# debbiemarkslab/BEAR

Measured on AMD Instinct MI355X. Metric: k-mer contexts/sec (DM-marginal+grad h), k=13, higher is better.
Workload: dtype f64

## Files before the change

### bear_amd/csrc/bear_count.hip

```cpp
#include <hip/hip_runtime.h>
#include <rocprim/device/device_radix_sort.hpp>
#include <rocprim/device/device_scan.hpp>
#include <stdint.h>

#include "../../include/bear_hip.h"
#include "bear_levels.h"

namespace {
thread_local int g_count_hip_error = 0;
#define CNT_TRY(expr)                    \
  do {                                   \
    hipError_t _e = (expr);              \
    if (_e != hipSuccess) {              \
      g_count_hip_error = (int)_e;       \
      st = BEAR_ERR_HIP;                 \
      goto done;                         \
    }                                    \
  } while (0)

template <int BITS, int W>
struct cnt_alphabet;
template <>
struct cnt_alphabet<3, 5> {
  static constexpr int MAX_LAG = 21;
// ... 288 lines not shown
  for (uint64_t i = (uint64_t)blockIdx.x * 256 + threadIdx.x; i < n; i += (uint64_t)gridDim.x * 256)
    flag[i] = (i == 0 || ((codes[i] ^ codes[i - 1]) & mask) != 0ull) ? 1u : 0u;
}
__global__ __launch_bounds__(256) void level_compact_kernel(const unsigned long long *__restrict__ codes, uint64_t n, unsigned long long mask,
                                                            unsigned long long fill, const uint32_t *__restrict__ flag,
                                                            uint32_t *__restrict__ scan_to_parent, unsigned long long *__restrict__ out_codes,
                                                            uint32_t *__restrict__ child_start, uint64_t n_runs) {
  for (uint64_t i = (uint64_t)blockIdx.x * 256 + threadIdx.x; i < n; i += (uint64_t)gridDim.x * 256) {
    const uint32_t run = scan_to_parent[i] - 1u;
    if (flag[i]) {
      out_codes[run] = (codes[i] & mask) | fill;
      child_start[run] = (uint32_t)i;
    }
    scan_to_parent[i] = run;
    if (i == 0) child_start[n_runs] = (uint32_t)n;
  }
}
}

namespace {
struct rec16 { unsigned long long a, b; };
struct rec16_less {
  __device__ __host__ bool operator()(const rec16 &x, const rec16 &y) const { return x.a < y.a || (x.a == y.a && x.b < y.b); }
};
template <typename T, typename Less>
int canonical_sort(T *d, uint64_t n, Less less, hipStream_t s) {
  int st = BEAR_OK;
  void *temp = nullptr;
  size_t tb = 0;
  T *out = nullptr;
  CNT_TRY(hipMalloc(&out, n * sizeof(T)));
  CNT_TRY(rocprim::merge_sort(nullptr, tb, d, out, n, less, s));
  CNT_TRY(hipMalloc(&temp, tb ? tb : 8));
  CNT_TRY(rocprim::merge_sort(temp, tb, d, out, n, less, s));
  CNT_TRY(hipMemcpyAsync(d, out, n * sizeof(T), hipMemcpyDeviceToDevice, s));
  CNT_TRY(hipStreamSynchronize(s));
done:
  if (temp) (void)hipFree(temp);
  if (out) (void)hipFree(out);
  return st;
}
}

int bear_canonical_order(void *records, uint64_t n, int width, hipStream_t s) {
  if (n < 2) return BEAR_OK;
  if (!records) return BEAR_ERR_INVALID_ARG;
  if (width == 16) return canonical_sort(static_cast<rec16 *>(records), n, rec16_less(), s);
  if (width == 8) return canonical_sort(static_cast<unsigned long long *>(records), n, rocprim::less<unsigned long long>(), s);
  if (width == 4) return canonical_sort(static_cast<uint32_t *>(records), n, rocprim::less<uint32_t>(), s);
  return BEAR_ERR_INVALID_ARG;
}

namespace {
__global__ __launch_bounds__(256) void window_keys_kernel(const unsigned long long *__restrict__ codes, uint64_t n, int shift, unsigned long long mask,
                                                          unsigned long long *__restrict__ keys, uint32_t *__restrict__ vals) {
  for (uint64_t i = (uint64_t)blockIdx.x * 256 + threadIdx.x; i < n; i += (uint64_t)gridDim.x * 256) {
    keys[i] = (codes[i] >> shift) & mask;
    vals[i] = (uint32_t)i;
  }
}
__global__ __launch_bounds__(256) void window_compact_kernel(const unsigned long long *__restrict__ keys, const uint32_t *__restrict__ perm, uint64_t n,
                                                             int shift, unsigned long long fill, const uint32_t *__restrict__ flag,
                                                             const uint32_t *__restrict__ scan, unsigned long long *__restrict__ out_codes,
                                                             uint32_t *__restrict__ child_start, uint32_t *__restrict__ row_of_context,
                                                             uint64_t n_runs) {
  for (uint64_t j = (uint64_t)blockIdx.x * 256 + threadIdx.x; j < n; j += (uint64_t)gridDim.x * 256) {
    const uint32_t run = scan[j] - 1u;
    if (flag[j]) {
      out_codes[run] = (keys[j] << shift) | fill;
      child_start[run] = (uint32_t)j;
    }
    row_of_context[perm[j]] = run;
    if (j == 0) child_start[n_runs] = (uint32_t)n;
  }
}
}

void bear_window_free(bear_window_dev *wt) {
  if (!wt) return;
  (void)hipFree(wt->codes);
  (void)hipFree(wt->row_of_context);
  (void)hipFree(wt->perm);
  (void)hipFree(wt->child_start);
  (void)hipFree(wt->rows);
  wt->codes = nullptr;
  wt->row_of_context = wt->perm = wt->child_start = nullptr;
  wt->rows = nullptr;
  wt->n = 0;
  wt->bytes = 0;
}

int bear_window_build(const unsigned long long *codes, uint64_t n_rows, int pos, int fw, bear_window_dev *out, hipStream_t s) {
  if (!codes || !out || n_rows == 0 || n_rows > 0xfffffffeull || pos < 0 || fw < 1 || pos + fw > 21) return BEAR_ERR_INVALID_ARG;
  int st = BEAR_OK;
  const int shift = 3 * pos;
  const unsigned long long mask = (1ull << (3 * fw)) - 1ull;
  unsigned long long fill = 0ull;
  for (int l = 0; l < 21; ++l)
    if (l < pos || l >= pos + fw) fill |= 5ull << (3 * l);
  unsigned long long *keys_in = nullptr, *keys = nullptr;
  uint32_t *vals_in = nullptr, *flag = nullptr, *scan = nullptr, n_runs = 0;
  void *temp = nullptr;
  size_t tb = 0, tb2 = 0;
  out->pos = pos;
  out->n = 0;
  out->codes = nullptr;
// ... 105 lines not shown
```

### bear_amd/csrc/bear_hip.hip

```cpp
#include "bear_host.h"
#include "kernels_finalize.h"
#include "kernels_rows.h"
#include "kernels_sorted.h"
#include "kernels_plan.h"
#include "kernels_synth.h"
#include "kernels_refmix.h"
#include "kernels_mixplan.h"
#include "kernels_sample.h"
#include "kernels_shuffle.h"
#include "kernels_refplan.h"

#ifdef PLN_STAMPS
#define PLN_DBG_ARG , ws->dbg
#else
#define PLN_DBG_ARG
#endif

thread_local int g_last_hip_error = 0;

extern "C" {

int bear_abi_version(void) { return BEAR_ABI_VERSION; }

const char *bear_strerror(int status) {
// ... 147 lines not shown
#define PRIOR_LAUNCH(AR, GRAD)                                                                                                          \
  hipLaunchKernelGGL((dm_prior_kernel<AR, GRAD>), dim3(grid), dim3(BEAR_THREADS), 0, s, counts, prior, n_rows, prm, grad_prior, \
                     reinterpret_cast<const double2 *>(ws->logtab), ws->partials)
    BEAR_DISPATCH_2(train_ar, grad_prior, PRIOR_LAUNCH);
#undef PRIOR_LAUNCH
  }
  HIP_TRY(hipGetLastError());
  hipLaunchKernelGGL(finalize_kernel, dim3(1), dim3(256), 0, s, ws->partials, grid, 2, out);
  HIP_TRY(hipGetLastError());
  return BEAR_OK;
}

int bear_dm_ref_f64(bear_ws *ws, const uint32_t *train, const uint32_t *ref, uint64_t n_rows,
                    double h_signed, double tau_signed, double nu_signed, double eps, int train_ar,
                    double *out, void *stream) {
  int st = check_ws(ws);
  if (st != BEAR_OK) return st;
  if (!out || (n_rows && (!train || !ref))) return BEAR_ERR_INVALID_ARG;
  if (misaligned(train) || misaligned(ref) || misaligned8(out)) return BEAR_ERR_INVALID_ARG;
  hipStream_t s = static_cast<hipStream_t>(stream);
  const bear_params prm = params_ref(h_signed, tau_signed, nu_signed, eps);
  const double2 *lt = reinterpret_cast<const double2 *>(ws->logtab);
  int grid = grid_rows(ws, n_rows);
  if (train_ar || getenv("BEAR_ROWS_KERNEL")) {
#define REF_LAUNCH(AR) hipLaunchKernelGGL((dm_ref_kernel<AR>), dim3(grid), dim3(BEAR_THREADS), 0, s, train, ref, n_rows, prm, lt, ws->partials)
    BEAR_DISPATCH_1(train_ar, REF_LAUNCH);
#undef REF_LAUNCH
  } else {
    grid = grid_sorted(ws, n_rows);
    hipLaunchKernelGGL(dm_ref_sorted_kernel, dim3(grid), dim3(SRT_THREADS), sizeof(srt_lds_r), s, train, ref, n_rows, prm, lt, ws->partials);
  }
  HIP_TRY(hipGetLastError());
  hipLaunchKernelGGL(finalize_kernel, dim3(1), dim3(256), 0, s, ws->partials, grid, 4, out);
  HIP_TRY(hipGetLastError());
  return BEAR_OK;
}

static void plan_free(bear_plan *p) {
  if (!p) return;
  (void)hipFree(p->tiles);
  (void)hipFree(p->stream);
  (void)hipFree(p->heavy_col);
  (void)hipFree(p->heavy_row);
  (void)hipFree(p->heavy_stop);
  (void)hipFree(p->hist);
  (void)hipFree(p->live);
  for (int k = 0; k < p->n_cnn_levels; ++k) bear_level_free(&p->cnn_levels[k]);
  for (int k = 0; k <= CNN_MAX_LAG; ++k)
    for (int q = 0; q < p->n_cnn_win[k]; ++q) bear_window_free(&p->cnn_win[k][q]);
  (void)hipFree(p->live2);
  (void)hipFree(p->tiles_p);
  (void)hipFree(p->tiles_u);
  (void)hipFree(p->ref_items);
  (void)hipFree(p->hist0_base);
  (void)hipFree(p->heavy0);
  (void)hipFree(p->sum0);
  delete p;
}

int bear_plan_create(bear_ws *ws, const uint32_t *counts, uint64_t n_rows, int ncol, bear_plan **out) {
  if (!out) return BEAR_ERR_INVALID_ARG;
  *out = nullptr;
  int st = check_ws(ws);
  if (st != BEAR_OK) return st;
  if ((ncol != 4 && ncol != 5) || (n_rows && !counts) || misaligned(counts)) return BEAR_ERR_INVALID_ARG;
  bear_plan *p = new (std::nothrow) bear_plan();
  if (!p) return BEAR_ERR_NOMEM;
  memset(p, 0, sizeof(*p));
  p->device = ws->device;
  p->ncol = ncol;
  p->n_rows = n_rows;
  p->counts = counts;
  hipError_t e = hipMalloc(&p->hist, sizeof(unsigned long long) * (2 * SRT_NKEY + PLN_NBIG + 1));
  if (e == hipSuccess) e = hipMemset(p->hist, 0, sizeof(unsigned long long) * (2 * SRT_NKEY + PLN_NBIG + 1));
  if (e != hipSuccess) {
    g_last_hip_error = (int)e;
    plan_free(p);
    return BEAR_ERR_HIP;
  }
  if (n_rows == 0) {
    *out = p;
    return BEAR_OK;
  }
  const uint64_t n_quads = (n_rows + PLN_QUAD - 1) / PLN_QUAD;
  uint8_t *d_quad = nullptr, *h_quad = nullptr;
  unsigned long long *d_cnt = nullptr;
  std::vector<pln_tile> tiles;
  e = hipMalloc(&d_quad, 3 * n_quads);
  if (e == hipSuccess) e = hipMalloc(&d_cnt, sizeof(unsigned long long) * 9);
  if (e == hipSuccess) e = hipMemset(d_cnt, 0, sizeof(unsigned long long) * 9);
  if (e == hipSuccess) {
    const int grid = grid_capped((n_quads + 255) / 256, (uint64_t)ws->num_cu * 8);
    hipLaunchKernelGGL(plan_scan_kernel, dim3(grid), dim3(256), 0, 0, counts, n_rows, ncol, d_quad, d_cnt, p->hist);
    e = hipGetLastError();
  }
  unsigned long long h_cnt[3] = {0, 0, 0}, h_total[3] = {0, 0, 0};
  if (e == hipSuccess) e = hipMemcpy(h_cnt, d_cnt, sizeof(h_cnt), hipMemcpyDeviceToHost);
  if (e == hipSuccess) e = hipMemcpy(h_total, d_cnt + 6, sizeof(h_total), hipMemcpyDeviceToHost);
  for (int k = 0; k < 3; ++k) p->count_total[k] = p->count_bound[k] = (double)h_total[k];
  uint64_t off16 = 0, n_tiles = 0;
  const char *cut_env = getenv("BEAR_PLAN_CUT");
  const bool host_cut = cut_env && cut_env[0] == 'h';
  if (e == hipSuccess && host_cut) {
    h_quad = (uint8_t *)malloc(3 * n_quads);
    if (!h_quad) e = hipErrorOutOfMemory;
    if (e == hipSuccess) e = hipMemcpy(h_quad, d_quad, 3 * n_quads, hipMemcpyDeviceToHost);
  }
  if (e == hipSuccess && host_cut) {
    uint64_t q = 0;
// ... 183 lines not shown

uint64_t bear_plan_tile_count(const bear_plan *plan) { return plan ? plan->n_tiles : 0; }

int bear_plan_tile_info(const bear_plan *plan, uint64_t first, uint64_t count, uint64_t *row0, uint32_t *rows, uint32_t *items,
                        uint64_t *stream_offset) {
  if (!plan || first + count > plan->n_tiles || (count && (!row0 || !rows || !items || !stream_offset))) return BEAR_ERR_INVALID_ARG;
  if (!count) return BEAR_OK;
  std::vector<pln_tile> h(count);
  int prev = 0;
  (void)hipGetDevice(&prev);
  (void)hipSetDevice(plan->device);
  const hipError_t e = hipMemcpy(h.data(), plan->tiles + first, sizeof(pln_tile) * count, hipMemcpyDeviceToHost);
  (void)hipSetDevice(prev);
  if (e != hipSuccess) {
    g_last_hip_error = (int)e;
    return BEAR_ERR_HIP;
  }
  for (uint64_t k = 0; k < count; ++k) {
    row0[k] = h[k].row0;
    rows[k] = h[k].rows_items >> 16;
    items[k] = h[k].rows_items & 0xffffu;
    stream_offset[k] = (uint64_t)h[k].off16 * 16;
  }
  return BEAR_OK;
}

int bear_plan_create_ref(bear_ws *ws, const uint32_t *train, const uint32_t *ref, uint64_t n_rows, bear_plan **out) {
  if (!out) return BEAR_ERR_INVALID_ARG;
  *out = nullptr;
  if ((n_rows && !ref) || misaligned(ref)) return BEAR_ERR_INVALID_ARG;
  bear_plan *p = nullptr;
  int st = bear_plan_create(ws, train, n_rows, 4, &p);
  if (st != BEAR_OK) return st;
  p->ref = ref;
  if (p->count_total[1] > 0.0 && (double)p->n_heavy[0] * 2.0 > p->count_total[1]) {
    (void)hipFree(p->tiles);
    (void)hipFree(p->stream);
    (void)hipFree(p->heavy_col);
    (void)hipFree(p->heavy_row);
    (void)hipFree(p->heavy_stop);
    p->tiles = nullptr;
    p->stream = nullptr;
    p->heavy_col = nullptr;
    p->heavy_row = nullptr;
    p->heavy_stop = nullptr;
    p->n_tiles = 0;
    p->n_heavy[0] = p->n_heavy[1] = p->n_heavy[2] = 0;
    p->rows_ref = 1;
    p->bytes = sizeof(unsigned long long) * (2 * SRT_NKEY + PLN_NBIG + 1);
    *out = p;
    return BEAR_OK;
  }
  unsigned long long *d_meta = nullptr;
  hipError_t e = hipMalloc(&d_meta, sizeof(unsigned long long) * 72);
  if (e == hipSuccess) e = hipMemset(d_meta, 0, sizeof(unsigned long long) * 72);
  if (e == hipSuccess) e = hipMalloc(&p->sum0, sizeof(double));
  if (e == hipSuccess) e = hipMemset(p->sum0, 0, sizeof(double));
  p->hist0_base = d_meta;
  unsigned long long h_meta[72];
  memset(h_meta, 0, sizeof(h_meta));
  const int grid = grid_capped((n_rows + 1023) / 1024, (uint64_t)ws->num_cu * 8);
  if (e == hipSuccess && n_rows) {
    hipLaunchKernelGGL(rpl_build_kernel, dim3(grid), dim3(256), 0, 0, train, ref, n_rows, 0, d_meta, d_meta + 32, d_meta + 64, p->sum0,
                       static_cast<rpl_item *>(nullptr), static_cast<uint32_t *>(nullptr));
    e = hipGetLastError();
    if (e == hipSuccess) e = hipMemcpy(h_meta, d_meta, sizeof(h_meta), hipMemcpyDeviceToHost);
  }
  if (e == hipSuccess) {
    unsigned long long run = 0, cur[RPL_NKEY];
    for (int k = 0; k < RPL_NKEY; ++k) {
      cur[k] = run;
      run += h_meta[k];
    }
    p->n_ref_items = run;
    p->n_heavy0 = h_meta[64];
    if (run) e = hipMalloc(&p->ref_items, sizeof(rpl_item) * run);
    if (e == hipSuccess && p->n_heavy0) e = hipMalloc(&p->heavy0, sizeof(uint32_t) * p->n_heavy0);
    if (e == hipSuccess) e = hipMemcpy(d_meta, cur, sizeof(cur), hipMemcpyHostToDevice);
    if (e == hipSuccess) e = hipMemset(d_meta + 64, 0, sizeof(unsigned long long));
    if (e == hipSuccess && n_rows && (run || p->n_heavy0)) {
      hipLaunchKernelGGL(rpl_build_kernel, dim3(grid), dim3(256), 0, 0, train, ref, n_rows, 1, d_meta, d_meta + 32, d_meta + 64, p->sum0,
                         p->ref_items, p->heavy0);
      e = hipGetLastError();
    }
    if (e == hipSuccess) e = hipDeviceSynchronize();
#ifdef BEAR_DET_BUILD
    for (int k = 0; k < RPL_NKEY && e == hipSuccess; ++k)
      if (bear_canonical_order(p->ref_items + cur[k], h_meta[k], 16, 0) != BEAR_OK) e = hipErrorUnknown;
    if (e == hipSuccess && bear_canonical_order(p->heavy0, p->n_heavy0, 4, 0) != BEAR_OK) e = hipErrorUnknown;
#endif
  }
  if (e != hipSuccess) {
    g_last_hip_error = (int)e;
    plan_free(p);
    return e == hipErrorOutOfMemory ? BEAR_ERR_NOMEM : BEAR_ERR_HIP;
  }
  p->hist0 = d_meta + 32;
  p->bytes += sizeof(rpl_item) * p->n_ref_items + sizeof(uint32_t) * p->n_heavy0 + sizeof(unsigned long long) * 72;
  *out = p;
  return BEAR_OK;
}

static int launch_prior_plan(bear_ws *ws, const bear_plan *plan, const double *prior, uint64_t n_rows, const bear_params &prm,
                             const double *theta, int train_ar, int prior_normalized, double *out, hipStream_t s) {
  const int grid = grid_plan(ws, plan->n_tiles);
  const double2 *lt = reinterpret_cast<const double2 *>(ws->logtab);
  const bear_step_io io = ws_io(ws, theta, BEAR_THETA_NET, out);
  if (train_ar)
    hipLaunchKernelGGL((dm_prior_plan_kernel<true, true>), dim3(grid), dim3(PLN_THREADS), sizeof(pln_lds_n), s, prior, n_rows, prm,
                       plan_view(plan), lt, ws->partials, io PLN_DBG_ARG);
  else if (prior_normalized)
    hipLaunchKernelGGL((dm_prior_plan_kernel<true, false>), dim3(grid), dim3(PLN_THREADS), sizeof(pln_lds_n), s, prior, n_rows, prm,
                       plan_view(plan), lt, ws->partials, io PLN_DBG_ARG);
  else
    hipLaunchKernelGGL((dm_prior_plan_kernel<false, false>), dim3(grid), dim3(PLN_THREADS), sizeof(pln_lds_n), s, prior, n_rows, prm,
                       plan_view(plan), lt, ws->partials, io PLN_DBG_ARG);
  HIP_TRY(hipGetLastError());
  return BEAR_OK;
}

int bear_dm_prior_plan_f64(bear_ws *ws, const bear_plan *plan, const uint32_t *counts, const double *prior,
                           uint64_t n_rows, double h_signed, double eps, int train_ar, int prior_normalized,
                           double *out, void *stream) {
  int st = check_ws(ws);
  if (st != BEAR_OK) return st;
  if (!plan || !out || (n_rows && (!counts || !prior))) return BEAR_ERR_INVALID_ARG;
  if (check_plan_step(ws, plan, counts, n_rows, 5, true) != BEAR_OK || misaligned(prior) || misaligned8(out)) return BEAR_ERR_INVALID_ARG;
  const bear_params prm = params_net(h_signed, eps);
  if (plan_is_rows(plan)) return launch_prior_rows(ws, plan, prior, prm, nullptr, train_ar, out, nullptr, static_cast<hipStream_t>(stream));
  return launch_prior_plan(ws, plan, prior, n_rows, prm, nullptr, train_ar, prior_normalized, out, static_cast<hipStream_t>(stream));
}

int launch_prior_plan_grad(bear_ws *ws, const bear_plan *plan, const double *prior, const bear_params &prm,
                                  const double *theta, int train_ar, int prior_normalized, double *out, double *grad_prior,
                                  hipStream_t s) {
  const int grid = grid_plan(ws, plan->n_tiles);
  const double2 *lt = reinterpret_cast<const double2 *>(ws->logtab);
  const pln_view pv = plan_view(plan);
  const bear_step_io io = ws_io(ws, theta, BEAR_THETA_NET, out);
  if (train_ar)
    hipLaunchKernelGGL((dm_prior_plan_grad_kernel<true, true>), dim3(grid), dim3(PLN_THREADS), sizeof(pln_lds_g), s, prior, prm, pv, lt,
                       grad_prior, ws->partials, io);
  else if (prior_normalized)
    hipLaunchKernelGGL(dm_prior_plan_grad_inplace_kernel, dim3(grid), dim3(PLN_THREADS), sizeof(pln_lds_gi), s, prior, prm, pv, lt,
                       grad_prior, ws->partials, io);
  else
    hipLaunchKernelGGL((dm_prior_plan_grad_kernel<false, false>), dim3(grid), dim3(PLN_THREADS), sizeof(pln_lds_g), s, prior, prm, pv, lt,
                       grad_prior, ws->partials, io);
  HIP_TRY(hipGetLastError());
  auto fixup_grid = [&](uint64_t nh) { return grid_capped((nh + 255) / 256, (uint64_t)ws->num_cu * 8); };
#define FIXUP(NORM, AR, ROWS, N) \
// ... 44 lines not shown
int bear_dm_refmix_plan_grad_f64(bear_ws *ws, const bear_plan *plan, const uint32_t *counts, const double *net_rows,
                                 const double *ref_rows, uint64_t n_rows, const double *h_signed_dev, const double *tau_signed_dev,
                                 const double *net_weight_signed_dev, double eps, int train_ar, double *out, double *grad_net_rows,
                                 void *stream) {
  int st = check_ws(ws);
  if (st != BEAR_OK) return st;
  if (!plan || !out || !h_signed_dev || !tau_signed_dev || !net_weight_signed_dev) return BEAR_ERR_INVALID_ARG;
  if (n_rows && (!counts || !net_rows || !ref_rows || !grad_net_rows)) return BEAR_ERR_INVALID_ARG;
  if (check_plan_step(ws, plan, counts, n_rows, 5) != BEAR_OK) return BEAR_ERR_INVALID_ARG;
  if (misaligned(net_rows) || misaligned(ref_rows) || misaligned(grad_net_rows) || misaligned8(out) || misaligned8(h_signed_dev) ||
      misaligned8(tau_signed_dev) || misaligned8(net_weight_signed_dev) || !(eps >= 0.0))
    return BEAR_ERR_INVALID_ARG;
  hipStream_t s = static_cast<hipStream_t>(stream);
  const int grid = grid_plan(ws, plan->n_tiles);
  const double2 *lt = reinterpret_cast<const double2 *>(ws->logtab);
  const pln_view pv = plan_view(plan);
  const bear_step_io io = ws_io(ws, nullptr, BEAR_THETA_REF, out);
#define MIX_LAUNCH(AR)                                                                                                            \
  hipLaunchKernelGGL(dm_refmix_plan_grad_kernel<AR>, dim3(grid), dim3(PLN_THREADS), sizeof(pln_lds_g), s, net_rows, ref_rows, \
                     h_signed_dev, tau_signed_dev, net_weight_signed_dev, eps, pv, lt, grad_net_rows, ws->partials, io)
  BEAR_DISPATCH_1(train_ar, MIX_LAUNCH);
#undef MIX_LAUNCH
  HIP_TRY(hipGetLastError());
  if (pv.n_heavy_col + pv.n_heavy_row) {
    const uint64_t nh = pv.n_heavy_col + pv.n_heavy_row;
    const int g2 = grid_capped((nh + 255) / 256, (uint64_t)ws->num_cu * 4);
#define MIX_FIXUP(AR)                                                                                                      \
  hipLaunchKernelGGL(dm_refmix_fixup_kernel<AR>, dim3(g2), dim3(256), 0, s, net_rows, ref_rows, h_signed_dev, tau_signed_dev, \
                     net_weight_signed_dev, eps, pv, lt, grad_net_rows)
    BEAR_DISPATCH_1(train_ar, MIX_FIXUP);
#undef MIX_FIXUP
    HIP_TRY(hipGetLastError());
  }
  return BEAR_OK;
}


static int launch_ref_plan(bear_ws *ws, const bear_plan *plan, const uint32_t *ref, uint64_t n_rows, const bear_params &prm,
                           const double *theta, int train_ar, double *out, hipStream_t s, const bear_apply_io &apply = NO_APPLY) {
  const double2 *lt = reinterpret_cast<const double2 *>(ws->logtab);
  const bear_step_io io = ws_io(ws, theta, BEAR_THETA_REF, out);
  int grid;
  if (plan->rows_ref) {
    if (plan->ref != ref) return BEAR_ERR_INVALID_ARG;
    grid = grid_dense(ws, n_rows);
#define REF_ROWS(AR) \
  hipLaunchKernelGGL(dm_ref_rows_kernel<AR>, dim3(grid), dim3(BEAR_THREADS), 0, s, plan->counts, ref, n_rows, prm, lt, ws->partials, io, apply)
    BEAR_DISPATCH_1(train_ar, REF_ROWS);
#undef REF_ROWS
  } else if (plan->ref) {
    if (plan->ref != ref) return BEAR_ERR_INVALID_ARG;
    rpl_view rv;
    rv.items = plan->ref_items;
    rv.n_items = plan->n_ref_items;
    rv.hist0 = plan->hist0;
    rv.heavy0 = plan->heavy0;
    rv.n_heavy0 = plan->n_heavy0;
    rv.sum0 = plan->sum0;
    const uint64_t units = (plan->n_ref_items + 63) / 64, want = (units + 3) / 4 + 2, cap = (uint64_t)ws->num_cu * (units > 131072 ? 6 : 4);
    grid = grid_capped(want, cap);
#define REF_ITEMS(AR) \
  hipLaunchKernelGGL(dm_ref_items_kernel<AR>, dim3(grid), dim3(256), 0, s, prm, rv, plan_view(plan), lt, ws->partials, io, apply)
    BEAR_DISPATCH_1(train_ar, REF_ITEMS);
#undef REF_ITEMS
  } else {
    grid = grid_plan(ws, plan->n_tiles);
#define REF_PLAN(AR)                                                                                                                     \
  hipLaunchKernelGGL(dm_ref_plan_kernel<AR>, dim3(grid), dim3(PLN_THREADS), sizeof(pln_lds_r), s, ref, n_rows, prm, plan_view(plan), lt, \
                     ws->partials, io, apply)
    BEAR_DISPATCH_1(train_ar, REF_PLAN);
#undef REF_PLAN
  }
  HIP_TRY(hipGetLastError());
  return BEAR_OK;
}

int bear_dm_ref_plan_f64(bear_ws *ws, const bear_plan *plan, const uint32_t *train, const uint32_t *ref,
                         uint64_t n_rows, double h_signed, double tau_signed, double nu_signed, double eps,
                         int train_ar, double *out, void *stream) {
  int st = check_ws(ws);
  if (st != BEAR_OK) return st;
  if (!plan || !out || (n_rows && (!train || !ref))) return BEAR_ERR_INVALID_ARG;
  if (check_plan_step(ws, plan, train, n_rows, 4) != BEAR_OK || misaligned(ref) || misaligned8(out)) return BEAR_ERR_INVALID_ARG;
  return launch_ref_plan(ws, plan, ref, n_rows, params_ref(h_signed, tau_signed, nu_signed, eps), nullptr, train_ar, out,
                         static_cast<hipStream_t>(stream));
}

static int ref_reduce(bear_ws *ws, const bear_plan *plan, const uint32_t *train, const uint32_t *ref, uint64_t n_rows, const double *theta,
                      double eps, int train_ar, double *packed, hipStream_t s, const bear_apply_io &apply) {
  int st = check_ws(ws);
  if (st != BEAR_OK) return st;
  if (!plan || !packed || !theta || !n_rows || !train || !ref) return BEAR_ERR_INVALID_ARG;
  if (check_plan_step(ws, plan, train, n_rows, 4) != BEAR_OK || misaligned(ref) || misaligned8(packed)) return BEAR_ERR_INVALID_ARG;
  return launch_ref_plan(ws, plan, ref, n_rows, params_eps(eps), theta, train_ar, packed, s, apply);
}

int bear_ref_train_reduce_f64(bear_ws *ws, const bear_plan *plan, const uint32_t *train, const uint32_t *ref, uint64_t n_rows,
                              const double *theta, double eps, int train_ar, double *packed, void *stream) {
  return ref_reduce(ws, plan, train, ref, n_rows, theta, eps, train_ar, packed, static_cast<hipStream_t>(stream), NO_APPLY);
}

int bear_ref_train_step_f64(bear_ws *ws, const bear_plan *plan, const uint32_t *train, const uint32_t *ref, uint64_t n_rows,
                            double *theta, double *adam_m, double *adam_v, double *adam_t, double eps, int train_ar,
                            double learning_rate, double scale, double *out, double *loss_buf, uint64_t loss_cap, void *stream) {
  if (!adam_m || !adam_v || !adam_t) return BEAR_ERR_INVALID_ARG;
  hipStream_t s = static_cast<hipStream_t>(stream);
  if (two_launch_step()) {
    int st = ref_reduce(ws, plan, train, ref, n_rows, theta, eps, train_ar, out, s, NO_APPLY);
    if (st != BEAR_OK) return st;
    return launch_train_apply(theta, 3, out, adam_m, adam_v, adam_t, learning_rate, scale, train_ar, loss_buf, loss_cap, s);
  }
  return ref_reduce(ws, plan, train, ref, n_rows, theta, eps, train_ar, out, s,
// ... 207 lines not shown
```

### bear_amd/csrc/bear_host.h

```cpp
#pragma once
#include <hip/hip_runtime.h>
#include <math.h>
#include <stdint.h>
#include <stdlib.h>
#include <string.h>

#include <initializer_list>
#include <new>
#include <vector>

#include "bear_common.h"
#include "bear_levels.h"
#include "plan_common.h"

#define BEAR_INTERNAL __attribute__((visibility("hidden")))

static inline int check_ws(const bear_ws *ws) {
  if (!ws) return BEAR_ERR_INVALID_ARG;
  int dev = -1;
  if (hipGetDevice(&dev) != hipSuccess) return BEAR_ERR_NO_DEVICE;
  if (dev != ws->device) return BEAR_ERR_WRONG_DEVICE;
  return BEAR_OK;
}

// ... 88 lines not shown
                                       double scale, int train_ar, double *loss_buf, uint64_t loss_cap) {
  bear_apply_io A;
  A.theta = theta;
  A.m = adam_m;
  A.v = adam_v;
  A.t_state = adam_t;
  A.loss_buf = loss_buf;
  A.loss_cap = (unsigned long long)loss_cap;
  A.lr = learning_rate;
  A.scale = scale;
  A.n_theta = n_theta;
  A.train_ar = train_ar;
  return A;
}

static inline bool two_launch_step() {
  const char *e = getenv("BEAR_AMD_TWO_LAUNCH_STEP");
  return e && e[0] && e[0] != '0';
}

struct rpl_item;
struct bear_plan {
  int device;
  int ncol;
  uint64_t n_rows;
  const uint32_t *counts;
  pln_tile *tiles;
  unsigned char *stream;
  pln_heavy_col *heavy_col;
  pln_heavy_row *heavy_row;
  uint64_t *heavy_stop;
  unsigned long long *hist;
  uint16_t *live;
  uint64_t n_tiles;
  uint64_t n_heavy[3];
  int rows_ref;
  uint64_t n_live_rows;
  double count_total[3];
  double count_bound[3];
  uint64_t bytes;
  bear_level_dev cnn_levels[CNN_MAX_LAG];
  int n_cnn_levels, cnn_lag, cnn_fw;
  bear_window_dev cnn_win[CNN_MAX_LAG + 1][CNN_MAX_WIN];
  int n_cnn_win[CNN_MAX_LAG + 1];
  int n_cnn_windows;
  const uint64_t *cnn_codes;
  uint16_t *live2;
  pln_tile *tiles_p, *tiles_u;
  uint64_t n_tiles_p, n_tiles_u;
  const uint64_t *pair_codes;
  int pair_lag;
  const uint32_t *ref;
  rpl_item *ref_items;
  uint64_t n_ref_items, n_heavy0;
  unsigned long long *hist0;
  unsigned long long *hist0_base;
  uint32_t *heavy0;
  double *sum0;
};

static inline pln_view plan_view(const bear_plan *p) {
  pln_view v;
  v.tiles = p->tiles;
  v.stream = p->stream;
  v.heavy_col = p->heavy_col;
  v.heavy_row = p->heavy_row;
  v.heavy_stop = p->heavy_stop;
  v.hist = p->hist;
  v.hist_big = p->hist + 2 * SRT_NKEY;
  v.big_in_hist = 1;
  v.live = p->live;
  v.live2 = p->live2;
  v.subset = 0;
  v.n_tiles = p->n_tiles;
  v.n_heavy_col = p->n_heavy[0];
  v.n_heavy_row = p->n_heavy[1];
  v.n_heavy_stop = p->n_heavy[2];
  return v;
}

#define PLAN_ROWS 15
static inline bool plan_is_rows(const bear_plan *p) { return p->ncol == PLAN_ROWS; }
static inline int check_plan_step(const bear_ws *ws, const bear_plan *plan, const uint32_t *counts, uint64_t n_rows, int ncol,
                                  bool or_rows = false) {
  if (plan->ncol != ncol && !(or_rows && plan_is_rows(plan))) return BEAR_ERR_INVALID_ARG;
  if (plan->counts != counts || plan->n_rows != n_rows || plan->device != ws->device) return BEAR_ERR_INVALID_ARG;
  return BEAR_OK;
}

BEAR_INTERNAL int linear_ws_setup(bear_ws *ws);
BEAR_INTERNAL int cnn_ws_setup(bear_ws *ws);
BEAR_INTERNAL int eval_ws_setup(bear_ws *ws);

extern "C" {
BEAR_INTERNAL int launch_prior_plan_grad(bear_ws *ws, const bear_plan *plan, const double *prior, const bear_params &prm,
                                         const double *theta, int train_ar, int prior_normalized, double *out, double *grad_prior,
                                         hipStream_t s);
BEAR_INTERNAL int launch_train_apply(double *theta, int n_theta, const double *packed, double *adam_m, double *adam_v, double *adam_t,
                                     double learning_rate, double scale, int train_ar, double *loss_buf, uint64_t loss_cap, hipStream_t s);
}
```

### bear_amd/csrc/bear_levels.h

```cpp
#pragma once
#include <hip/hip_runtime.h>
#include <stdint.h>

#define CNN_MAX_LAG 21
#define CNN_MAX_WIN 6

struct bear_level_dev {
  uint64_t n;
  int letters;
  unsigned long long *codes;
  uint32_t *parent_of_below;
  uint32_t *child_start;
  double *rows;
  uint64_t bytes;
};

struct bear_window_dev {
  int pos;
  uint64_t n;
  unsigned long long *codes;
  uint32_t *row_of_context;
  uint32_t *perm;
  uint32_t *child_start;
  double *rows;
  uint64_t bytes;
};
int bear_window_build(const unsigned long long *codes, uint64_t n_rows, int pos, int fw, bear_window_dev *out, hipStream_t stream);
void bear_window_free(bear_window_dev *wt);

int bear_level_build(const unsigned long long *codes_below, uint64_t n_below, int letters, bear_level_dev *out, hipStream_t stream);
void bear_level_free(bear_level_dev *lv);

int bear_canonical_order(void *records, uint64_t n, int width, hipStream_t stream);
```

### bear_amd/csrc/kernels_refplan.h

```cpp
#pragma once
#include "kernels_plan.h"

#define RPL_NKEY 32
#define RPL_HEAVY_KEY 24

struct rpl_item {
  uint32_t c, rb;
  double R;
};
static_assert(sizeof(rpl_item) == 16, "one 16-byte lane load per record");

struct rpl_view {
  const rpl_item *items;
  uint64_t n_items;
  const unsigned long long *hist0;
  const uint32_t *heavy0;
  uint64_t n_heavy0;
  const double *sum0;
};

__global__ __launch_bounds__(256) void rpl_build_kernel(const uint32_t *__restrict__ train, const uint32_t *__restrict__ ref, uint64_t n_rows,
                                                        int fill, unsigned long long *__restrict__ bucket,
                                                        unsigned long long *__restrict__ hist0, unsigned long long *__restrict__ n_heavy0,
                                                        double *__restrict__ sum0, rpl_item *__restrict__ items,
                                                        uint32_t *__restrict__ heavy0) {
  constexpr int RPT = 4;
  __shared__ uint32_t s_bucket[RPL_NKEY], s_hist0[RPL_NKEY];
  __shared__ unsigned long long s_at[RPL_NKEY];
  __shared__ double s_sum;
  const uint32_t tid = threadIdx.x;
  const uint64_t per_block = (n_rows + gridDim.x - 1) / gridDim.x;
  const uint64_t r_begin = (uint64_t)blockIdx.x * per_block, r_end = r_begin + per_block < n_rows ? r_begin + per_block : n_rows;
  for (uint64_t base = r_begin; base < r_end; base += 256u * RPT) {
    if (tid < RPL_NKEY) s_bucket[tid] = s_hist0[tid] = 0u;
    if (tid == 0) s_sum = 0.0;
    __syncthreads();
    uint32_t c[RPT][4], rb[RPT][4], rank[RPT][4];
    double R[RPT];
    double my_sum = 0.0;
#pragma unroll
    for (int k = 0; k < RPT; ++k) {
      const uint64_t row = base + tid + 256u * k;
      R[k] = -1.0;
#pragma unroll
      for (int b = 0; b < 4; ++b) c[k][b] = rb[k][b] = rank[k][b] = 0u;
      if (row < r_end) {
        uint64_t rs = 0;
#pragma unroll
        for (int b = 0; b < 4; ++b) {
          c[k][b] = train[row * 5 + b];
          rb[k][b] = ref[row * 5 + b];
          rs += rb[k][b];
        }
        R[k] = (double)rs;
#pragma unroll
        for (int b = 0; b < 4; ++b) {
          if (c[k][b] == 0u) continue;
          if (rs == 0) {
            my_sum += (double)c[k][b];
            if (c[k][b] <= SRT_CL) {
              if (!fill) atomicAdd(&s_hist0[c[k][b] - 1], 1u);
            } else if (fill) {
              heavy0[atomicAdd(n_heavy0, 1ull)] = c[k][b];
            } else {
              atomicAdd(n_heavy0, 1ull);
            }
          } else {
            const uint32_t key = (c[k][b] > SRT_CL ? SRT_CL + 1u : c[k][b]) - 1u;
            rank[k][b] = atomicAdd(&s_bucket[key], 1u);
          }
        }
      }
    }
    if (!fill && my_sum != 0.0) atomicAdd(&s_sum, my_sum);
    __syncthreads();
    if (tid < RPL_NKEY && !fill) {
      if (s_bucket[tid]) atomicAdd(&bucket[tid], (unsigned long long)s_bucket[tid]);
      if (s_hist0[tid]) atomicAdd(&hist0[tid], (unsigned long long)s_hist0[tid]);
    }
    if (!fill && tid == 0 && s_sum != 0.0) atomicAdd(sum0, s_sum);
    if (fill) {
      if (tid < RPL_NKEY) s_at[tid] = s_bucket[tid] ? atomicAdd(&bucket[tid], (unsigned long long)s_bucket[tid]) : 0ull;
      __syncthreads();
#pragma unroll
      for (int k = 0; k < RPT; ++k) {
        if (!(R[k] > 0.0)) continue;
#pragma unroll
        for (int b = 0; b < 4; ++b) {
          if (c[k][b] == 0u) continue;
          const uint32_t key = (c[k][b] > SRT_CL ? SRT_CL + 1u : c[k][b]) - 1u;
          rpl_item it;
          it.c = c[k][b];
          it.rb = rb[k][b];
          it.R = R[k];
          items[s_at[key] + rank[k][b]] = it;
        }
      }
    }
    __syncthreads();
  }
}

template <bool AR>
__global__ __launch_bounds__(256) void dm_ref_items_kernel(bear_params prm_arg, rpl_view rv, pln_view pv, const double2 *__restrict__ logtab_g,
                                                           double *__restrict__ partials, const bear_step_io io, const bear_apply_io apply) {
  __shared__ double2 s_log[BEAR_LOGTAB_N];
  const bear_params prm = bear_params_of(prm_arg, io);
  const uint32_t tid = threadIdx.x, lane = tid & 63u;
  const double u = prm.inv_h, eps = prm.eps;
  const double A = u + 5.0 * eps;
  const double x4 = prm.nw * prm.V * u + eps;
  const double VU = prm.V * u;
  const double tau = prm.tau;
  const double w2c = tau * (eps + 0.25 * VU);
  const double nwV = prm.nw * prm.V;
  double acc[4] = {0.0, 0.0, 0.0, 0.0};
  if (tid < BEAR_LOGTAB_N) s_log[tid] = logtab_g[tid];
  __syncthreads();
  auto alpha_from = [&](double rb, double R) {
    const double dev = __builtin_fma(rb + eps, bear_rcp(R), -0.25);
    return __builtin_fma(__builtin_fma(prm.E, dev, 0.25), VU, eps);
  };
  auto accumulate = [&](double x, double m, const bear_dp &o) {
    const double w1 = eps - x, P = m * o.P;
    acc[0] = __builtin_fma(m, o.D, acc[0]);
    acc[1] = __builtin_fma(w1, P, acc[1]);
    acc[2] = __builtin_fma(__builtin_fma(-tau, x, w2c), P, acc[2]);
    acc[3] = __builtin_fma(nwV * w1, P, acc[3]);
  };
  auto accumulate_ar = [&](double rb, double R, double c) {
    const double dev = __builtin_fma(rb + eps, bear_rcp(R), -0.25);
    const double f = __builtin_fma(prm.E, dev, 0.25) * prm.V;
    const double p = f + eps;
    const double dLdf = c * bear_rcp(p);
    acc[0] = __builtin_fma(c, bear_log_tab(p, s_log), acc[0]);
    acc[2] = __builtin_fma(dLdf, -prm.tauE * dev * prm.V, acc[2]);
    acc[3] = __builtin_fma(dLdf, -nwV * f, acc[3]);
  };
  const uint64_t n_units = (rv.n_items + 63u) >> 6;
  const uint64_t wave_g = ((uint64_t)blockIdx.x * 256u + tid) >> 6, n_waves = ((uint64_t)gridDim.x * 256u) >> 6;
  for (uint64_t un = wave_g; un < n_units; un += n_waves) {
    const uint64_t i = un * 64u + lane;
    rpl_item it;
    it.c = 0u;
    it.rb = 0u;
    it.R = 1.0;
    if (i < rv.n_items) it = rv.items[i];
    const double R = it.R + 4.0 * eps;
    if (AR) {
      if (it.c) accumulate_ar((double)it.rb, R, (double)it.c);
      continue;
    }
    const bool heavy = it.c > SRT_CL;
    const uint32_t cc = heavy ? SRT_CL + 1u : it.c;
    const uint32_t occ = (un + 1u) * 64u <= rv.n_items ? 64u : (uint32_t)(rv.n_items - un * 64u);
    const uint32_t cmin = occ == 64u ? (uint32_t)__builtin_amdgcn_readlane((int)cc, 0) : 0u;
    const uint32_t cmax = (uint32_t)__builtin_amdgcn_readlane((int)cc, (int)(occ - 1u));
    const double x[1] = {alpha_from((double)it.rb, R)};
    const uint32_t ci[1] = {heavy ? 0u : it.c};
    bear_dp o[1];
    srt_light<1>(x, ci, cmin > SRT_CL ? SRT_CL : cmin, cmax > SRT_CL ? SRT_CL : cmax, s_log, o);
    if (__builtin_amdgcn_ballot_w64(heavy)) {
      if (heavy) o[0] = srt_general_fast(x[0], (double)it.c, s_log);
    }
    if (it.c) accumulate(x[0], 1.0, o[0]);
  }
  const uint64_t gtid = (uint64_t)blockIdx.x * 256u + tid, gsz = (uint64_t)gridDim.x * 256u;
  const double R0 = 4.0 * eps;
  if (AR) {
    if (gtid == 0) accumulate_ar(0.0, R0, rv.sum0[0]);
    const double f4 = nwV, p4 = f4 + eps;
    double c4sum = 0.0;
    if (blockIdx.x == 0 && tid < SRT_CL) c4sum = (double)(tid + 1) * (double)pv.hist[SRT_NKEY + tid];
    for (uint64_t i = gtid; i < pv.n_heavy_stop; i += gsz) c4sum += (double)pv.heavy_stop[i];
    acc[0] = __builtin_fma(c4sum, bear_log_tab(p4, s_log), acc[0]);
    acc[3] = __builtin_fma(c4sum * bear_rcp(p4), nwV * (1.0 - f4), acc[3]);
    __syncthreads();
    block_finish<4>(acc, partials, io, apply);
    return;
  }
  const double x0 = alpha_from(0.0, R0);
  if (blockIdx.x == 0 && tid < SRT_CL) {
    const double m = (double)rv.hist0[tid];
    if (m != 0.0) accumulate(x0, m, srt_general_fast(x0, (double)(tid + 1), s_log));
  }
  for (uint64_t i = gtid; i < rv.n_heavy0; i += gsz) accumulate(x0, 1.0, srt_general_fast(x0, (double)rv.heavy0[i], s_log));
  for (uint64_t i = gtid; i < pv.n_heavy_row; i += gsz) {
    const double n = pv.heavy_row[i].n;
    if (pln_in_big_hist(pv, n)) continue;
    const bear_dp o = srt_general_fast(A, n, s_log);
    acc[0] -= o.D;
    acc[1] = __builtin_fma(u, o.P, acc[1]);
  }
  pln_big_totals(pv, A, u, gtid, gsz, s_log, acc[0], acc[1]);
  for (uint64_t i = gtid; i < pv.n_heavy_stop; i += gsz) {
    const bear_dp o = srt_general_fast(x4, (double)pv.heavy_stop[i], s_log);
    acc[0] += o.D;
    acc[1] = __builtin_fma(eps - x4, o.P, acc[1]);
    acc[3] = __builtin_fma(VU * nwV, o.P, acc[3]);
  }
  if (blockIdx.x == 1 % gridDim.x && tid < SRT_CL) {
    const double mn = (double)pv.hist[tid], m4 = (double)pv.hist[SRT_NKEY + tid];
    const bear_dp on = srt_general_fast(A, (double)(tid + 1), s_log), o4 = srt_general_fast(x4, (double)(tid + 1), s_log);
    acc[0] -= mn * on.D;
    acc[1] = __builtin_fma(u * mn, on.P, acc[1]);
    const double P4 = m4 * o4.P;
    acc[0] += m4 * o4.D;
    acc[1] = __builtin_fma(eps - x4, P4, acc[1]);
    acc[3] = __builtin_fma(VU * nwV, P4, acc[3]);
  }
  __syncthreads();
  block_finish<4>(acc, partials, io, apply);
}
```

Before: 136.8 billion.

## Deduplicate reference items into merged records with multiplicities

Plan creation now collects all reference items, including zero-row ones, into one list. The list is sorted with a capped-count comparator and identical (c, rb/R) records are merged into unique items carrying a multiplicity, with light zero-row counts binned through a histogram. The per-call kernel then evaluates each unique item once, weighted by its multiplicity, and drops the separate hist0/heavy0/sum0 paths. It also retunes the grid sizing to include the heavy counts and caps it at 4 blocks per CU. This moves work to plan time and adds a multiplicity load per item, and it changes the order of floating-point summation.

```diff
diff --git a/bear_amd/csrc/bear_count.hip b/bear_amd/csrc/bear_count.hip
--- a/bear_amd/csrc/bear_count.hip
+++ b/bear_amd/csrc/bear_count.hip
@@ -364,6 +364,84 @@
 }
 
 namespace {
+struct rec16_capped_less {
+  uint32_t cap;
+  __device__ __host__ bool operator()(const rec16 &x, const rec16 &y) const {
+    const uint32_t cx = (uint32_t)x.a, cy = (uint32_t)y.a;
+    const uint32_t kx = cx > cap ? cap + 1u : cx, ky = cy > cap ? cap + 1u : cy;
+    return kx < ky || (kx == ky && rec16_less()(x, y));
+  }
+};
+__global__ __launch_bounds__(256) void merge_flag_kernel(const rec16 *__restrict__ rec, uint64_t n, unsigned long long *__restrict__ flag) {
+  for (uint64_t i = (uint64_t)blockIdx.x * 256 + threadIdx.x; i < n; i += (uint64_t)gridDim.x * 256)
+    flag[i] = (i == 0 || rec[i].a != rec[i - 1].a || rec[i].b != rec[i - 1].b) ? 1ull : 0ull;
+}
+__global__ __launch_bounds__(256) void merge_compact_kernel(const rec16 *__restrict__ rec, uint64_t n, const unsigned long long *__restrict__ scan,
+                                                            rec16 *__restrict__ out, unsigned long long *__restrict__ start, uint64_t n_runs) {
+  for (uint64_t i = (uint64_t)blockIdx.x * 256 + threadIdx.x; i < n; i += (uint64_t)gridDim.x * 256) {
+    if (i == 0 || scan[i] != scan[i - 1]) {
+      out[scan[i] - 1ull] = rec[i];
+      start[scan[i] - 1ull] = i;
+    }
+    if (i == 0) start[n_runs] = n;
+  }
+}
+__global__ __launch_bounds__(256) void merge_mult_kernel(const rec16 *__restrict__ out, const unsigned long long *__restrict__ start, uint64_t n_runs,
+                                                         uint32_t cap, const unsigned long long *__restrict__ light0,
+                                                         unsigned long long *__restrict__ mult) {
+  for (uint64_t r = (uint64_t)blockIdx.x * 256 + threadIdx.x; r < n_runs; r += (uint64_t)gridDim.x * 256) {
+    const rec16 x = out[r];
+    const bool bin = x.b == 0ull && x.a >= 1ull && x.a <= (unsigned long long)cap;
+    mult[r] = bin ? light0[x.a - 1ull] : start[r + 1] - start[r];
+  }
+}
+}
+
+int bear_merge_records(void *records, uint64_t n, uint32_t cap, const unsigned long long *light0, void **out_items,
+                       unsigned long long **out_mult, uint64_t *n_out, hipStream_t s) {
+  if (!out_items || !out_mult || !n_out) return BEAR_ERR_INVALID_ARG;
+  *out_items = nullptr;
+  *out_mult = nullptr;
+  *n_out = 0;
+  if (n == 0) return BEAR_OK;
+  if (!records || !light0) return BEAR_ERR_INVALID_ARG;
+  rec16 *rec = static_cast<rec16 *>(records), *merged = nullptr;
+  int st = n < 2 ? BEAR_OK : canonical_sort(rec, n, rec16_capped_less{cap}, s);
+  if (st != BEAR_OK) return st;
+  unsigned long long *scan = nullptr, *start = nullptr, *mult = nullptr, n_runs = 0;
+  void *temp = nullptr;
+  size_t tb = 0;
+  CNT_TRY(hipMalloc(&scan, n * sizeof(unsigned long long)));
+  hipLaunchKernelGGL(merge_flag_kernel, dim3(grid_for(n)), dim3(256), 0, s, rec, n, scan);
+  CNT_TRY(hipGetLastError());
+  CNT_TRY(rocprim::inclusive_scan(nullptr, tb, scan, scan, n, rocprim::plus<unsigned long long>(), s));
+  CNT_TRY(hipMalloc(&temp, tb ? tb : 8));
+  CNT_TRY(rocprim::inclusive_scan(temp, tb, scan, scan, n, rocprim::plus<unsigned long long>(), s));
+  CNT_TRY(hipMemcpyAsync(&n_runs, scan + (n - 1), sizeof(n_runs), hipMemcpyDeviceToHost, s));
+  CNT_TRY(hipStreamSynchronize(s));
+  CNT_TRY(hipMalloc(&merged, n_runs * sizeof(rec16)));
+  CNT_TRY(hipMalloc(&mult, n_runs * sizeof(unsigned long long)));
+  CNT_TRY(hipMalloc(&start, (n_runs + 1) * sizeof(unsigned long long)));
+  hipLaunchKernelGGL(merge_compact_kernel, dim3(grid_for(n)), dim3(256), 0, s, rec, n, scan, merged, start, n_runs);
+  CNT_TRY(hipGetLastError());
+  hipLaunchKernelGGL(merge_mult_kernel, dim3(grid_for(n_runs)), dim3(256), 0, s, merged, start, n_runs, cap, light0, mult);
+  CNT_TRY(hipGetLastError());
+  CNT_TRY(hipStreamSynchronize(s));
+  *out_items = merged;
+  *out_mult = mult;
+  *n_out = n_runs;
+  merged = nullptr;
+  mult = nullptr;
+done:
+  if (temp) (void)hipFree(temp);
+  if (scan) (void)hipFree(scan);
+  if (start) (void)hipFree(start);
+  if (merged) (void)hipFree(merged);
+  if (mult) (void)hipFree(mult);
+  return st;
+}
+
+namespace {
 __global__ __launch_bounds__(256) void window_keys_kernel(const unsigned long long *__restrict__ codes, uint64_t n, int shift, unsigned long long mask,
                                                           unsigned long long *__restrict__ keys, uint32_t *__restrict__ vals) {
   for (uint64_t i = (uint64_t)blockIdx.x * 256 + threadIdx.x; i < n; i += (uint64_t)gridDim.x * 256) {
diff --git a/bear_amd/csrc/bear_hip.hip b/bear_amd/csrc/bear_hip.hip
--- a/bear_amd/csrc/bear_hip.hip
+++ b/bear_amd/csrc/bear_hip.hip
@@ -223,9 +223,7 @@
   (void)hipFree(p->tiles_p);
   (void)hipFree(p->tiles_u);
   (void)hipFree(p->ref_items);
-  (void)hipFree(p->hist0_base);
-  (void)hipFree(p->heavy0);
-  (void)hipFree(p->sum0);
+  (void)hipFree(p->ref_mult);
   delete p;
 }
 
@@ -515,51 +513,42 @@
     return BEAR_OK;
   }
   unsigned long long *d_meta = nullptr;
-  hipError_t e = hipMalloc(&d_meta, sizeof(unsigned long long) * 72);
-  if (e == hipSuccess) e = hipMemset(d_meta, 0, sizeof(unsigned long long) * 72);
-  if (e == hipSuccess) e = hipMalloc(&p->sum0, sizeof(double));
-  if (e == hipSuccess) e = hipMemset(p->sum0, 0, sizeof(double));
-  p->hist0_base = d_meta;
-  unsigned long long h_meta[72];
+  rpl_item *d_list = nullptr;
+  hipError_t e = hipMalloc(&d_meta, sizeof(unsigned long long) * 32);
+  if (e == hipSuccess) e = hipMemset(d_meta, 0, sizeof(unsigned long long) * 32);
+  unsigned long long h_meta[32];
   memset(h_meta, 0, sizeof(h_meta));
   const int grid = grid_capped((n_rows + 1023) / 1024, (uint64_t)ws->num_cu * 8);
   if (e == hipSuccess && n_rows) {
-    hipLaunchKernelGGL(rpl_build_kernel, dim3(grid), dim3(256), 0, 0, train, ref, n_rows, 0, d_meta, d_meta + 32, d_meta + 64, p->sum0,
-                       static_cast<rpl_item *>(nullptr), static_cast<uint32_t *>(nullptr));
+    hipLaunchKernelGGL(rpl_build_kernel, dim3(grid), dim3(256), 0, 0, train, ref, n_rows, 0, d_meta, d_meta + 8, static_cast<rpl_item *>(nullptr));
     e = hipGetLastError();
     if (e == hipSuccess) e = hipMemcpy(h_meta, d_meta, sizeof(h_meta), hipMemcpyDeviceToHost);
   }
   if (e == hipSuccess) {
-    unsigned long long run = 0, cur[RPL_NKEY];
-    for (int k = 0; k < RPL_NKEY; ++k) {
-      cur[k] = run;
-      run += h_meta[k];
-    }
-    p->n_ref_items = run;
-    p->n_heavy0 = h_meta[64];
-    if (run) e = hipMalloc(&p->ref_items, sizeof(rpl_item) * run);
-    if (e == hipSuccess && p->n_heavy0) e = hipMalloc(&p->heavy0, sizeof(uint32_t) * p->n_heavy0);
-    if (e == hipSuccess) e = hipMemcpy(d_meta, cur, sizeof(cur), hipMemcpyHostToDevice);
-    if (e == hipSuccess) e = hipMemset(d_meta + 64, 0, sizeof(unsigned long long));
-    if (e == hipSuccess && n_rows && (run || p->n_heavy0)) {
-      hipLaunchKernelGGL(rpl_build_kernel, dim3(grid), dim3(256), 0, 0, train, ref, n_rows, 1, d_meta, d_meta + 32, d_meta + 64, p->sum0,
-                         p->ref_items, p->heavy0);
+    unsigned long long n_list = h_meta[0];
+    for (int k = 0; k < SRT_CL; ++k) n_list += h_meta[8 + k] != 0ull;
+    if (n_list) e = hipMalloc(&d_list, sizeof(rpl_item) * n_list);
+    if (e == hipSuccess) e = hipMemset(d_meta, 0, sizeof(unsigned long long));
+    if (e == hipSuccess && n_list) {
+      hipLaunchKernelGGL(rpl_build_kernel, dim3(grid), dim3(256), 0, 0, train, ref, n_rows, 1, d_meta, d_meta + 8, d_list);
       e = hipGetLastError();
     }
     if (e == hipSuccess) e = hipDeviceSynchronize();
-#ifdef BEAR_DET_BUILD
-    for (int k = 0; k < RPL_NKEY && e == hipSuccess; ++k)
-      if (bear_canonical_order(p->ref_items + cur[k], h_meta[k], 16, 0) != BEAR_OK) e = hipErrorUnknown;
-    if (e == hipSuccess && bear_canonical_order(p->heavy0, p->n_heavy0, 4, 0) != BEAR_OK) e = hipErrorUnknown;
-#endif
-  }
+    if (e == hipSuccess) {
+      void *merged = nullptr;
+      const int mst = bear_merge_records(d_list, n_list, SRT_CL, d_meta + 8, &merged, &p->ref_mult, &p->n_ref_items, 0);
+      p->ref_items = static_cast<rpl_item *>(merged);
+      if (mst != BEAR_OK) e = mst == BEAR_ERR_NOMEM ? hipErrorOutOfMemory : hipErrorUnknown;
+    }
+  }
+  (void)hipFree(d_list);
+  (void)hipFree(d_meta);
   if (e != hipSuccess) {
     g_last_hip_error = (int)e;
     plan_free(p);
     return e == hipErrorOutOfMemory ? BEAR_ERR_NOMEM : BEAR_ERR_HIP;
   }
-  p->hist0 = d_meta + 32;
-  p->bytes += sizeof(rpl_item) * p->n_ref_items + sizeof(uint32_t) * p->n_heavy0 + sizeof(unsigned long long) * 72;
+  p->bytes += (sizeof(rpl_item) + sizeof(unsigned long long)) * p->n_ref_items;
   *out = p;
   return BEAR_OK;
 }
@@ -710,12 +699,10 @@
     if (plan->ref != ref) return BEAR_ERR_INVALID_ARG;
     rpl_view rv;
     rv.items = plan->ref_items;
+    rv.mult = plan->ref_mult;
     rv.n_items = plan->n_ref_items;
-    rv.hist0 = plan->hist0;
-    rv.heavy0 = plan->heavy0;
-    rv.n_heavy0 = plan->n_heavy0;
-    rv.sum0 = plan->sum0;
-    const uint64_t units = (plan->n_ref_items + 63) / 64, want = (units + 3) / 4 + 2, cap = (uint64_t)ws->num_cu * (units > 131072 ? 6 : 4);
+    const uint64_t units = (plan->n_ref_items + 63) / 64 + (plan->n_heavy[1] + plan->n_heavy[2]) / 512;
+    const uint64_t want = (units + 3) / 4 + 2, cap = (uint64_t)ws->num_cu * 4;
     grid = grid_capped(want, cap);
 #define REF_ITEMS(AR) \
   hipLaunchKernelGGL(dm_ref_items_kernel<AR>, dim3(grid), dim3(256), 0, s, prm, rv, plan_view(plan), lt, ws->partials, io, apply)
diff --git a/bear_amd/csrc/bear_host.h b/bear_amd/csrc/bear_host.h
--- a/bear_amd/csrc/bear_host.h
+++ b/bear_amd/csrc/bear_host.h
@@ -164,11 +164,8 @@
   int pair_lag;
   const uint32_t *ref;
   rpl_item *ref_items;
-  uint64_t n_ref_items, n_heavy0;
-  unsigned long long *hist0;
-  unsigned long long *hist0_base;
-  uint32_t *heavy0;
-  double *sum0;
+  unsigned long long *ref_mult;
+  uint64_t n_ref_items;
 };
 
 static inline pln_view plan_view(const bear_plan *p) {
diff --git a/bear_amd/csrc/bear_levels.h b/bear_amd/csrc/bear_levels.h
--- a/bear_amd/csrc/bear_levels.h
+++ b/bear_amd/csrc/bear_levels.h
@@ -32,3 +32,6 @@
 void bear_level_free(bear_level_dev *lv);
 
 int bear_canonical_order(void *records, uint64_t n, int width, hipStream_t stream);
+
+int bear_merge_records(void *records, uint64_t n, uint32_t cap, const unsigned long long *light0, void **out_items,
+                       unsigned long long **out_mult, uint64_t *n_out, hipStream_t stream);
diff --git a/bear_amd/csrc/kernels_refplan.h b/bear_amd/csrc/kernels_refplan.h
--- a/bear_amd/csrc/kernels_refplan.h
+++ b/bear_amd/csrc/kernels_refplan.h
@@ -1,8 +1,5 @@
 #pragma once
 #include "kernels_plan.h"
-
-#define RPL_NKEY 32
-#define RPL_HEAVY_KEY 24
 
 struct rpl_item {
   uint32_t c, rb;
@@ -12,36 +9,37 @@
 
 struct rpl_view {
   const rpl_item *items;
+  const unsigned long long *mult;
   uint64_t n_items;
-  const unsigned long long *hist0;
-  const uint32_t *heavy0;
-  uint64_t n_heavy0;
-  const double *sum0;
 };
 
 __global__ __launch_bounds__(256) void rpl_build_kernel(const uint32_t *__restrict__ train, const uint32_t *__restrict__ ref, uint64_t n_rows,
-                                                        int fill, unsigned long long *__restrict__ bucket,
-                                                        unsigned long long *__restrict__ hist0, unsigned long long *__restrict__ n_heavy0,
-                                                        double *__restrict__ sum0, rpl_item *__restrict__ items,
-                                                        uint32_t *__restrict__ heavy0) {
+                                                        int fill, unsigned long long *__restrict__ n_list,
+                                                        unsigned long long *__restrict__ light0, rpl_item *__restrict__ items) {
   constexpr int RPT = 4;
-  __shared__ uint32_t s_bucket[RPL_NKEY], s_hist0[RPL_NKEY];
-  __shared__ unsigned long long s_at[RPL_NKEY];
-  __shared__ double s_sum;
+  __shared__ uint32_t s_n, s_light0[SRT_CL];
+  __shared__ unsigned long long s_at;
   const uint32_t tid = threadIdx.x;
   const uint64_t per_block = (n_rows + gridDim.x - 1) / gridDim.x;
   const uint64_t r_begin = (uint64_t)blockIdx.x * per_block, r_end = r_begin + per_block < n_rows ? r_begin + per_block : n_rows;
+  if (fill && blockIdx.x == 0 && tid < SRT_CL && light0[tid]) {
+    rpl_item it;
+    it.c = tid + 1u;
+    it.rb = 0u;
+    it.R = 0.0;
+    items[atomicAdd(n_list, 1ull)] = it;
+  }
   for (uint64_t base = r_begin; base < r_end; base += 256u * RPT) {
-    if (tid < RPL_NKEY) s_bucket[tid] = s_hist0[tid] = 0u;
-    if (tid == 0) s_sum = 0.0;
+    if (tid < SRT_CL) s_light0[tid] = 0u;
+    if (tid == 0) s_n = 0u;
     __syncthreads();
     uint32_t c[RPT][4], rb[RPT][4], rank[RPT][4];
     double R[RPT];
-    double my_sum = 0.0;
+    auto listed = [&](int k, int b) { return c[k][b] != 0u && (R[k] > 0.0 || c[k][b] > SRT_CL); };
 #pragma unroll
     for (int k = 0; k < RPT; ++k) {
       const uint64_t row = base + tid + 256u * k;
-      R[k] = -1.0;
+      R[k] = 0.0;
 #pragma unroll
       for (int b = 0; b < 4; ++b) c[k][b] = rb[k][b] = rank[k][b] = 0u;
       if (row < r_end) {
@@ -55,45 +53,28 @@
         R[k] = (double)rs;
 #pragma unroll
         for (int b = 0; b < 4; ++b) {
-          if (c[k][b] == 0u) continue;
-          if (rs == 0) {
-            my_sum += (double)c[k][b];
-            if (c[k][b] <= SRT_CL) {
-              if (!fill) atomicAdd(&s_hist0[c[k][b] - 1], 1u);
-            } else if (fill) {
-              heavy0[atomicAdd(n_heavy0, 1ull)] = c[k][b];
-            } else {
-              atomicAdd(n_heavy0, 1ull);
-            }
-          } else {
-            const uint32_t key = (c[k][b] > SRT_CL ? SRT_CL + 1u : c[k][b]) - 1u;
-            rank[k][b] = atomicAdd(&s_bucket[key], 1u);
-          }
+          if (listed(k, b)) rank[k][b] = atomicAdd(&s_n, 1u);
+          else if (c[k][b] != 0u && !fill) atomicAdd(&s_light0[c[k][b] - 1u], 1u);
         }
       }
     }
-    if (!fill && my_sum != 0.0) atomicAdd(&s_sum, my_sum);
     __syncthreads();
-    if (tid < RPL_NKEY && !fill) {
-      if (s_bucket[tid]) atomicAdd(&bucket[tid], (unsigned long long)s_bucket[tid]);
-      if (s_hist0[tid]) atomicAdd(&hist0[tid], (unsigned long long)s_hist0[tid]);
-    }
-    if (!fill && tid == 0 && s_sum != 0.0) atomicAdd(sum0, s_sum);
-    if (fill) {
-      if (tid < RPL_NKEY) s_at[tid] = s_bucket[tid] ? atomicAdd(&bucket[tid], (unsigned long long)s_bucket[tid]) : 0ull;
+    if (!fill) {
+      if (tid < SRT_CL && s_light0[tid]) atomicAdd(&light0[tid], (unsigned long long)s_light0[tid]);
+      if (tid == 0 && s_n) atomicAdd(n_list, (unsigned long long)s_n);
+    } else {
+      if (tid == 0) s_at = s_n ? atomicAdd(n_list, (unsigned long long)s_n) : 0ull;
       __syncthreads();
 #pragma unroll
       for (int k = 0; k < RPT; ++k) {
-        if (!(R[k] > 0.0)) continue;
 #pragma unroll
         for (int b = 0; b < 4; ++b) {
-          if (c[k][b] == 0u) continue;
-          const uint32_t key = (c[k][b] > SRT_CL ? SRT_CL + 1u : c[k][b]) - 1u;
+          if (!listed(k, b)) continue;
           rpl_item it;
           it.c = c[k][b];
           it.rb = rb[k][b];
           it.R = R[k];
-          items[s_at[key] + rank[k][b]] = it;
+          items[s_at + rank[k][b]] = it;
         }
       }
     }
@@ -145,10 +126,14 @@
     it.c = 0u;
     it.rb = 0u;
     it.R = 1.0;
-    if (i < rv.n_items) it = rv.items[i];
+    double m = 0.0;
+    if (i < rv.n_items) {
+      it = rv.items[i];
+      m = (double)rv.mult[i];
+    }
     const double R = it.R + 4.0 * eps;
     if (AR) {
-      if (it.c) accumulate_ar((double)it.rb, R, (double)it.c);
+      if (it.c) accumulate_ar((double)it.rb, R, m * (double)it.c);
       continue;
     }
     const bool heavy = it.c > SRT_CL;
@@ -163,12 +148,10 @@
     if (__builtin_amdgcn_ballot_w64(heavy)) {
       if (heavy) o[0] = srt_general_fast(x[0], (double)it.c, s_log);
     }
-    if (it.c) accumulate(x[0], 1.0, o[0]);
+    if (it.c) accumulate(x[0], m, o[0]);
   }
   const uint64_t gtid = (uint64_t)blockIdx.x * 256u + tid, gsz = (uint64_t)gridDim.x * 256u;
-  const double R0 = 4.0 * eps;
   if (AR) {
-    if (gtid == 0) accumulate_ar(0.0, R0, rv.sum0[0]);
     const double f4 = nwV, p4 = f4 + eps;
     double c4sum = 0.0;
     if (blockIdx.x == 0 && tid < SRT_CL) c4sum = (double)(tid + 1) * (double)pv.hist[SRT_NKEY + tid];
@@ -179,12 +162,6 @@
     block_finish<4>(acc, partials, io, apply);
     return;
   }
-  const double x0 = alpha_from(0.0, R0);
-  if (blockIdx.x == 0 && tid < SRT_CL) {
-    const double m = (double)rv.hist0[tid];
-    if (m != 0.0) accumulate(x0, m, srt_general_fast(x0, (double)(tid + 1), s_log));
-  }
-  for (uint64_t i = gtid; i < rv.n_heavy0; i += gsz) accumulate(x0, 1.0, srt_general_fast(x0, (double)rv.heavy0[i], s_log));
   for (uint64_t i = gtid; i < pv.n_heavy_row; i += gsz) {
     const double n = pv.heavy_row[i].n;
     if (pln_in_big_hist(pv, n)) continue;
```

After: 136.7 billion. Within noise of the previous version (-0.1%).
